# imironhead/ml_super_resolution

Measured on AMD Instinct MI355X. Metric: VDSR-20 training patches/sec (41x41, batch 256 per GPU); fwd HR megapixels/sec alongside, higher is better.
Workload: dtype f32; 1 GPU; BASELINE configs[2]: VDSR 20-layer 3x3x64 residual, RGB, batch 256x41x41 per GPU, fwd+bwd+TF-Adam, random-init weights; global_batch=256, patch=41, parallelism=dp1

## Files before the change

### ml_super_resolution_amd/csrc/conv_narrow.hip

```cpp
#include "launchers.h"
namespace srx {
typedef float f32x3 __attribute__((ext_vector_type(3)));
typedef unsigned u32x3v __attribute__((ext_vector_type(3)));

template <int CTRL>
__device__ __forceinline__ float dpp_add(float v) {
    const int moved = __builtin_amdgcn_update_dpp(0, __float_as_int(v), CTRL, 0xf, 0xf, false);
    return v + __int_as_float(moved);
}

struct PixWalk {
    int n, oh, ow;
    __device__ __forceinline__ void init(unsigned p, int OH, int OW) {
        const unsigned t = p / (unsigned)OW;
        ow = (int)(p - t * (unsigned)OW);
        n = (int)(t / (unsigned)OH);
        oh = (int)(t - (unsigned)n * (unsigned)OH);
    }
    __device__ __forceinline__ void step16(int OH, int OW) { step(16, OH, OW); }
    __device__ __forceinline__ void step(int d, int OH, int OW) {
        ow += d;
        while (ow >= OW) {
            ow -= OW;
            oh += 1;
            if (oh == OH) { oh = 0; n += 1; }
        }
    }
};
template <int KH, int KW>
__device__ __forceinline__ void tap_offsets(int (&off)[KH * KW], const PixWalk& q, bool live, int H, int W, int pad_t, int pad_l,
                                            int PB, int lane_b) {
    const int centre = ((q.n * H + q.oh - pad_t) * W + (q.ow - pad_l)) * PB + lane_b;
    bool rok[KH], cok[KW];
#pragma unroll
    for (int kh = 0; kh < KH; ++kh) rok[kh] = live && (unsigned)(q.oh + kh - pad_t) < (unsigned)H;
#pragma unroll
    for (int kw = 0; kw < KW; ++kw) cok[kw] = (unsigned)(q.ow + kw - pad_l) < (unsigned)W;
#pragma unroll
    for (int kh = 0; kh < KH; ++kh)
#pragma unroll
        for (int kw = 0; kw < KW; ++kw)
            off[kh * KW + kw] = (rok[kh] && cok[kw]) ? centre + (kh * W + kw) * PB : kOobOffset;
}

template <int KH, int KW, int CIN, int CO>
__global__ __launch_bounds__(256) void conv_narrow_kernel(const ConvArgs a, long total_px, int iters) {
    static_assert(CIN == 64, "16 lanes x 4 channels per pixel");
    constexpr int TAPS = KH * KW;
    const int c4 = threadIdx.x & 15;
    const int sub = threadIdx.x >> 4;
    float wr[TAPS][4][CO];
#pragma unroll
    for (int t = 0; t < TAPS; ++t)
#pragma unroll
        for (int e = 0; e < 4; ++e)
#pragma unroll
            for (int c = 0; c < CO; ++c) wr[t][e][c] = a.w[((size_t)t * CIN + 4 * c4 + e) * CO + c];
    float bias[CO];
#pragma unroll
    for (int c = 0; c < CO; ++c) bias[c] = a.bias ? a.bias[c] : 0.0f;
    const __amdgpu_buffer_rsrc_t xrs = __builtin_amdgcn_make_buffer_rsrc(const_cast<float*>(a.x), 0,
                                                                         a.N * a.H * a.W * CIN * 4, 0x00020000);
    const unsigned p0 = blockIdx.x * (unsigned)iters * 16u + sub;
    PixWalk q;
    q.init(p0 < (unsigned)total_px ? p0 : 0u, a.OH, a.OW);
    for (int it = 0; it < iters; ++it, q.step16(a.OH, a.OW)) {
        const unsigned p = p0 + (unsigned)it * 16u;
        const bool live = p < (unsigned)total_px;
        int off[TAPS];
        tap_offsets<KH, KW>(off, q, live, a.H, a.W, a.pad_t, a.pad_l, CIN * 4, 16 * c4);
        f32x4 v[TAPS];
#pragma unroll
        for (int tp = 0; tp < TAPS; ++tp)
            v[tp] = __builtin_bit_cast(f32x4, __builtin_amdgcn_raw_buffer_load_b128(xrs, off[tp], 0, 0));
        float acc[CO];
#pragma unroll
        for (int c = 0; c < CO; ++c) acc[c] = 0.0f;
#pragma unroll
        for (int tp = 0; tp < TAPS; ++tp)
#pragma unroll
            for (int e = 0; e < 4; ++e)
#pragma unroll
                for (int c = 0; c < CO; ++c) acc[c] = fmaf(v[tp][e], wr[tp][e][c], acc[c]);
#pragma unroll
        for (int c = 0; c < CO; ++c) {
            float r = acc[c];
            r = dpp_add<0xB1>(r);
            r = dpp_add<0x4E>(r);
            r = dpp_add<0x124>(r);
            r = dpp_add<0x128>(r);
            acc[c] = r;
        }
        if (live && c4 < CO) {
            float r = (c4 == 0) ? acc[0] : (c4 == 1 ? acc[1 < CO ? 1 : 0] : acc[2 < CO ? 2 : 0]);
            r = act_apply(r + ((c4 == 0) ? bias[0] : (c4 == 1 ? bias[1 < CO ? 1 : 0] : bias[2 < CO ? 2 : 0])), a.act);
            const size_t o = (size_t)p * CO + c4;
            if (a.skip) r += a.skip[o];
            if (a.post_relu) r = act_apply(r, a.post_relu);
            a.y[o] = r;
        }
    }
}

template <int KH, int KW, bool NOUT, int CW = 64>
__global__ __launch_bounds__(256) void wgrad_narrow_kernel(const WgradArgs a, long total_px, int iters) {
    constexpr int TAPS = KH * KW, CN = 3;
    constexpr int LPP = CW / 4;
    constexpr int PPI = 256 / LPP;
    constexpr int NB = NOUT ? CN : 4;
    constexpr int NV = TAPS * 4 * CN + NB;
    __shared__ float red[4 * NV * LPP];
    const int c4 = threadIdx.x & (LPP - 1);
    const int sub = threadIdx.x / LPP;
    const int wave = threadIdx.x >> 6;
    float acc[NV];
#pragma unroll
    for (int i = 0; i < NV; ++i) acc[i] = 0.0f;
    const __amdgpu_buffer_rsrc_t xrs = __builtin_amdgcn_make_buffer_rsrc(
        const_cast<float*>(a.x), 0, a.N * a.H * a.W * (NOUT ? CW : CN) * 4, 0x00020000);
    const __amdgpu_buffer_rsrc_t drs = __builtin_amdgcn_make_buffer_rsrc(
        const_cast<float*>(a.dpre), 0, a.N * a.OH * a.OW * (NOUT ? CN : CW) * 4, 0x00020000);
    const unsigned p0 = blockIdx.x * (unsigned)iters * (unsigned)PPI + sub;
    PixWalk q;
    q.init(p0 < (unsigned)total_px ? p0 : 0u, a.OH, a.OW);
    for (int it = 0; it < iters; ++it, q.step(PPI, a.OH, a.OW)) {
        const unsigned p = p0 + (unsigned)it * (unsigned)PPI;
        const bool live = p < (unsigned)total_px;
        int off[TAPS];
        tap_offsets<KH, KW>(off, q, live, a.H, a.W, a.pad_t, a.pad_l, (NOUT ? CW : CN) * 4, NOUT ? 16 * c4 : 0);
        if constexpr (NOUT) {
            const f32x3 d = __builtin_bit_cast(f32x3, __builtin_amdgcn_raw_buffer_load_b96(drs, live ? (int)(p * CN * 4) : kOobOffset, 0, 0));
            f32x4 v[TAPS];
#pragma unroll
            for (int tp = 0; tp < TAPS; ++tp)
                v[tp] = __builtin_bit_cast(f32x4, __builtin_amdgcn_raw_buffer_load_b128(xrs, off[tp], 0, 0));
#pragma unroll
            for (int tp = 0; tp < TAPS; ++tp)
#pragma unroll
                for (int e = 0; e < 4; ++e)
#pragma unroll
                    for (int c = 0; c < CN; ++c) acc[(tp * 4 + e) * CN + c] = fmaf(v[tp][e], d[c], acc[(tp * 4 + e) * CN + c]);
#pragma unroll
            for (int c = 0; c < CN; ++c) acc[TAPS * 4 * CN + c] += d[c];
        } else {
            const f32x4 d = __builtin_bit_cast(f32x4, __builtin_amdgcn_raw_buffer_load_b128(
                drs, live ? (int)((p * CW + 4 * c4) * 4) : kOobOffset, 0, 0));
            f32x3 v[TAPS];
#pragma unroll
            for (int tp = 0; tp < TAPS; ++tp)
                v[tp] = __builtin_bit_cast(f32x3, __builtin_amdgcn_raw_buffer_load_b96(xrs, off[tp], 0, 0));
#pragma unroll
            for (int tp = 0; tp < TAPS; ++tp)
#pragma unroll
                for (int cn = 0; cn < CN; ++cn)
#pragma unroll
                    for (int e = 0; e < 4; ++e) acc[(tp * CN + cn) * 4 + e] = fmaf(v[tp][cn], d[e], acc[(tp * CN + cn) * 4 + e]);
#pragma unroll
            for (int e = 0; e < 4; ++e) acc[TAPS * 4 * CN + e] += d[e];
        }
    }
#pragma unroll
    for (int i = 0; i < NV; ++i) {
        float r = acc[i];
#pragma unroll
        for (int o = LPP; o < 64; o <<= 1) r += __shfl_xor(r, o);
        if (sub % (64 / LPP) == 0) red[(wave * NV + i) * LPP + c4] = r;
    }
    __syncthreads();
    float* part = a.part + (size_t)blockIdx.x * a.part_stride;
    const int wn = TAPS * CW * CN;
    for (int q = threadIdx.x; q < NV * LPP; q += 256) {
        const int i = q / LPP, l = q % LPP;
        const float r = (red[(0 * NV + i) * LPP + l] + red[(1 * NV + i) * LPP + l]) +
                        (red[(2 * NV + i) * LPP + l] + red[(3 * NV + i) * LPP + l]);
        if (i < TAPS * 4 * CN) {
            int idx;
            if constexpr (NOUT) {
                const int c = i % CN, te = i / CN, e = te & 3, tp = te >> 2;
                idx = (tp * CW + 4 * l + e) * CN + c;
            } else {
                const int e = i & 3, tc = i >> 2;
                idx = tc * CW + 4 * l + e;
            }
            part[idx] = r;
        } else {
            const int b = i - TAPS * 4 * CN;
            if constexpr (NOUT) {
                if (l == 0) part[wn + b] = r;
            } else {
                part[wn + 4 * l + b] = r;
            }
        }
    }
}

bool launch_wgrad_narrow(const ConvKey& k, const WgradArgs& a, int grid, hipStream_t s, hipError_t* err) {
    if (k.kh != 3 || k.kw != 3) return false;
    const bool nout = a.Cin == 64 && a.Cout == 3, nin = a.Cin == 3 && a.Cout == 64, nin32 = a.Cin == 3 && a.Cout == 32;
    if (!nout && !nin && !nin32) return false;
    const long total = (long)a.N * a.OH * a.OW;
    if (total >= (1L << 31) - 4096 || (long)a.N * a.H * a.W * 64 * 4 >= (1L << 31) - 4096 || total * 64 * 4 >= (1L << 31) - 4096)
        return false;
    const long ppi = nin32 ? 32 : 16;
    const int iters = (int)((total + ppi * grid - 1) / (ppi * grid));
    if (nout)
        hipLaunchKernelGGL((wgrad_narrow_kernel<3, 3, true>), dim3(grid), dim3(256), 0, s, a, total, iters);
    else if (nin)
        hipLaunchKernelGGL((wgrad_narrow_kernel<3, 3, false>), dim3(grid), dim3(256), 0, s, a, total, iters);
    else
        hipLaunchKernelGGL((wgrad_narrow_kernel<3, 3, false, 32>), dim3(grid), dim3(256), 0, s, a, total, iters);
    *err = hipGetLastError();
    return true;
}

bool launch_conv_narrow(const ConvKey& k, const ConvArgs& a, hipStream_t s, hipError_t* err) {
    if (k.wt || a.Cout != 3 || a.mask) return false;
    if ((long)a.N * a.H * a.W * a.Cin * 4 >= (1L << 31) - 4096) return false;
    const long total = (long)a.N * a.OH * a.OW;
    int iters = 16;
    while (iters > 1 && total / (16L * iters) < 2048) iters >>= 1;
    const long blocks = (total + 16L * iters - 1) / (16L * iters);
    if (total >= (1L << 31) - 4096) return false;
    if (k.kh == 3 && k.kw == 3 && a.Cin == 64) {
        hipLaunchKernelGGL((conv_narrow_kernel<3, 3, 64, 3>), dim3((unsigned)blocks), dim3(256), 0, s, a, total, iters);
    } else {
        return false;
    }
    *err = hipGetLastError();
    return true;
}
}
```

Baseline: 19530 patches/s.

## Walk output rows in runs with sliding 3-column input window for narrow convs

Replaces the per-pixel narrow conv forward (64->3) and the 64<->3 wgrad kernels with row-run walkers. Each 16-lane group processes a contiguous run of up to 14 output pixels and keeps a rotating window of input columns, so each input column is loaded once per run instead of three times. Loads are software-prefetched two steps ahead. Inner FMAs use packed v_pk_fma_f32 written as inline asm, and outputs are written with buffer stores. This cuts redundant global loads and FMA instruction count, in exchange for more registers and hand-written asm with manual s_nop hazard handling.

```diff
diff --git a/ml_super_resolution_amd/csrc/conv_narrow.hip b/ml_super_resolution_amd/csrc/conv_narrow.hip
--- a/ml_super_resolution_amd/csrc/conv_narrow.hip
+++ b/ml_super_resolution_amd/csrc/conv_narrow.hip
@@ -1,4 +1,6 @@
 #include "launchers.h"
+#include <type_traits>
+#include <utility>
 namespace srx {
 typedef float f32x3 __attribute__((ext_vector_type(3)));
 typedef unsigned u32x3v __attribute__((ext_vector_type(3)));
@@ -43,62 +45,182 @@
             off[kh * KW + kw] = (rok[kh] && cok[kw]) ? centre + (kh * W + kw) * PB : kOobOffset;
 }
 
-template <int KH, int KW, int CIN, int CO>
-__global__ __launch_bounds__(256) void conv_narrow_kernel(const ConvArgs a, long total_px, int iters) {
-    static_assert(CIN == 64, "16 lanes x 4 channels per pixel");
-    constexpr int TAPS = KH * KW;
+constexpr int kRunMax = 14;
+
+struct RunPlan {
+    int nruns, steps;
+    unsigned total_runs;
+};
+inline RunPlan plan_runs(long rows, int OW) {
+    RunPlan r;
+    r.nruns = (OW + kRunMax - 1) / kRunMax;
+    r.steps = (OW + r.nruns - 1) / r.nruns;
+    r.total_runs = (unsigned)(rows * r.nruns);
+    return r;
+}
+
+struct Run {
+    int row, n, oh, ow0, len;
+    __device__ __forceinline__ void init(unsigned r, const RunPlan& rp, int OH, int OW) {
+        const bool live = r < rp.total_runs;
+        const unsigned rr = live ? r : 0u;
+        const unsigned rw = rr / (unsigned)rp.nruns;
+        row = (int)rw;
+        ow0 = (int)(rr - rw * (unsigned)rp.nruns) * rp.steps;
+        n = (int)(rw / (unsigned)OH);
+        oh = row - n * OH;
+        len = live ? min(rp.steps, OW - ow0) : 0;
+        if (len < 0) len = 0;
+    }
+};
+
+template <typename V>
+__device__ __forceinline__ V load_px(__amdgpu_buffer_rsrc_t rs, int off) {
+    if constexpr (sizeof(V) == 16)
+        return __builtin_bit_cast(V, __builtin_amdgcn_raw_buffer_load_b128(rs, off, 0, 0));
+    else
+        return __builtin_bit_cast(V, __builtin_amdgcn_raw_buffer_load_b96(rs, off, 0, 0));
+}
+
+template <typename V, int PB>
+struct ColWalk {
+    int o[3], iw;
+    bool rok[3];
+    __device__ __forceinline__ void init(const Run& q, int H, int W, int pad_t, int pad_l, int lane_b) {
+        iw = q.ow0 - pad_l;
+#pragma unroll
+        for (int kh = 0; kh < 3; ++kh) {
+            const int ih = q.oh + kh - pad_t;
+            rok[kh] = q.len > 0 && (unsigned)ih < (unsigned)H;
+            o[kh] = (int)((((unsigned)q.n * (unsigned)H + (unsigned)ih) * (unsigned)W + (unsigned)iw) * (unsigned)PB + (unsigned)lane_b);
+        }
+    }
+    __device__ __forceinline__ void next(__amdgpu_buffer_rsrc_t rs, int W, V (&col)[3], bool on = true) {
+        const bool cok = on && (unsigned)iw < (unsigned)W;
+#pragma unroll
+        for (int kh = 0; kh < 3; ++kh) {
+            col[kh] = load_px<V>(rs, (rok[kh] && cok) ? o[kh] : kOobOffset);
+            o[kh] += PB;
+        }
+        iw += 1;
+    }
+};
+
+template <int HALF, bool LAST = false>
+__device__ __forceinline__ void pk_fma_bcast(f32x2& acc, f32x2 a, f32x2 b) {
+    if constexpr (HALF == 0) {
+        if constexpr (LAST) asm volatile("v_pk_fma_f32 %0, %1, %2, %0 op_sel_hi:[0,1,1]\n\ts_nop 1" : "+v"(acc) : "v"(a), "v"(b));
+        else asm volatile("v_pk_fma_f32 %0, %1, %2, %0 op_sel_hi:[0,1,1]" : "+v"(acc) : "v"(a), "v"(b));
+    } else {
+        if constexpr (LAST) asm volatile("v_pk_fma_f32 %0, %1, %2, %0 op_sel:[1,0,0] op_sel_hi:[1,1,1]\n\ts_nop 1" : "+v"(acc) : "v"(a), "v"(b));
+        else asm volatile("v_pk_fma_f32 %0, %1, %2, %0 op_sel:[1,0,0] op_sel_hi:[1,1,1]" : "+v"(acc) : "v"(a), "v"(b));
+    }
+}
+__device__ __forceinline__ f32x2 lo2(f32x4 v) { return __builtin_shufflevector(v, v, 0, 1); }
+__device__ __forceinline__ f32x2 hi2(f32x4 v) { return __builtin_shufflevector(v, v, 2, 3); }
+__device__ __forceinline__ f32x2 lo2(f32x3 v) { return __builtin_shufflevector(v, v, 0, 1); }
+__device__ __forceinline__ f32x2 hi2(f32x3 v) { return __builtin_shufflevector(v, v, 2, -1); }
+
+__device__ __forceinline__ void loads_issued() { asm volatile("" ::: "memory"); }
+
+constexpr int kAhead = 2;
+constexpr int kSlots = 3 + kAhead;
+template <int S>
+using StepPhase = std::integral_constant<int, S>;
+template <typename F, int... I>
+__device__ __forceinline__ void walk_steps_impl(int steps, F&& f, std::integer_sequence<int, I...>) {
+    for (int s = 0;; s += kSlots) {
+        bool done = false;
+        ((done = done || (f(StepPhase<I>{}, s + I), s + I + 1 >= steps)), ...);
+        if (done) break;
+    }
+}
+template <typename F>
+__device__ __forceinline__ void walk_steps(int steps, F&& f) {
+    walk_steps_impl(steps, f, std::make_integer_sequence<int, kSlots>{});
+}
+
+__global__ __launch_bounds__(256) void conv_narrow_rows_kernel(const ConvArgs a, const RunPlan rp, int iters) {
+    constexpr int PB = 64 * 4;
     const int c4 = threadIdx.x & 15;
     const int sub = threadIdx.x >> 4;
-    float wr[TAPS][4][CO];
-#pragma unroll
-    for (int t = 0; t < TAPS; ++t)
-#pragma unroll
-        for (int e = 0; e < 4; ++e)
-#pragma unroll
-            for (int c = 0; c < CO; ++c) wr[t][e][c] = a.w[((size_t)t * CIN + 4 * c4 + e) * CO + c];
-    float bias[CO];
-#pragma unroll
-    for (int c = 0; c < CO; ++c) bias[c] = a.bias ? a.bias[c] : 0.0f;
-    const __amdgpu_buffer_rsrc_t xrs = __builtin_amdgcn_make_buffer_rsrc(const_cast<float*>(a.x), 0,
-                                                                         a.N * a.H * a.W * CIN * 4, 0x00020000);
-    const unsigned p0 = blockIdx.x * (unsigned)iters * 16u + sub;
-    PixWalk q;
-    q.init(p0 < (unsigned)total_px ? p0 : 0u, a.OH, a.OW);
-    for (int it = 0; it < iters; ++it, q.step16(a.OH, a.OW)) {
-        const unsigned p = p0 + (unsigned)it * 16u;
-        const bool live = p < (unsigned)total_px;
-        int off[TAPS];
-        tap_offsets<KH, KW>(off, q, live, a.H, a.W, a.pad_t, a.pad_l, CIN * 4, 16 * c4);
-        f32x4 v[TAPS];
-#pragma unroll
-        for (int tp = 0; tp < TAPS; ++tp)
-            v[tp] = __builtin_bit_cast(f32x4, __builtin_amdgcn_raw_buffer_load_b128(xrs, off[tp], 0, 0));
-        float acc[CO];
-#pragma unroll
-        for (int c = 0; c < CO; ++c) acc[c] = 0.0f;
-#pragma unroll
-        for (int tp = 0; tp < TAPS; ++tp)
-#pragma unroll
-            for (int e = 0; e < 4; ++e)
-#pragma unroll
-                for (int c = 0; c < CO; ++c) acc[c] = fmaf(v[tp][e], wr[tp][e][c], acc[c]);
-#pragma unroll
-        for (int c = 0; c < CO; ++c) {
-            float r = acc[c];
-            r = dpp_add<0xB1>(r);
-            r = dpp_add<0x4E>(r);
-            r = dpp_add<0x124>(r);
-            r = dpp_add<0x128>(r);
-            acc[c] = r;
-        }
-        if (live && c4 < CO) {
-            float r = (c4 == 0) ? acc[0] : (c4 == 1 ? acc[1 < CO ? 1 : 0] : acc[2 < CO ? 2 : 0]);
-            r = act_apply(r + ((c4 == 0) ? bias[0] : (c4 == 1 ? bias[1 < CO ? 1 : 0] : bias[2 < CO ? 2 : 0])), a.act);
-            const size_t o = (size_t)p * CO + c4;
-            if (a.skip) r += a.skip[o];
+    f32x2 w01[9][4];
+    float w2[9][4];
+#pragma unroll
+    for (int t = 0; t < 9; ++t)
+#pragma unroll
+        for (int e = 0; e < 4; ++e) {
+            const float* wp = a.w + ((size_t)t * 64 + 4 * c4 + e) * 3;
+            w01[t][e] = f32x2{wp[0], wp[1]};
+            w2[t][e] = wp[2];
+        }
+    const float bias_l = (a.bias && c4 < 3) ? a.bias[c4] : 0.0f;
+    const int ybytes = a.N * a.OH * a.OW * 3 * 4;
+    const __amdgpu_buffer_rsrc_t xrs = __builtin_amdgcn_make_buffer_rsrc(const_cast<float*>(a.x), 0, a.N * a.H * a.W * PB, 0x00020000);
+    const __amdgpu_buffer_rsrc_t yrs = __builtin_amdgcn_make_buffer_rsrc(a.y, 0, ybytes, 0x00020000);
+    const __amdgpu_buffer_rsrc_t srs = __builtin_amdgcn_make_buffer_rsrc(const_cast<float*>(a.skip), 0, a.skip ? ybytes : 0, 0x00020000);
+    for (int it = 0; it < iters; ++it) {
+        Run q;
+        q.init((blockIdx.x * (unsigned)iters + (unsigned)it) * 16u + sub, rp, a.OH, a.OW);
+        ColWalk<f32x4, PB> cw;
+        cw.init(q, a.H, a.W, a.pad_t, a.pad_l, 16 * c4);
+        f32x4 win[kSlots][3];
+#pragma unroll
+        for (int c = 0; c < kSlots - 1; ++c) cw.next(xrs, a.W, win[c], c < rp.steps + 2);
+        int yo = ((q.row * a.OW + q.ow0) * 3 + c4) * 4;
+        int left = (c4 < 3) ? q.len : 0;
+        int so_ahead = yo, left_ahead = left;
+        auto next_skip = [&]() {
+            const float v = __builtin_bit_cast(float, __builtin_amdgcn_raw_buffer_load_b32(srs, left_ahead > 0 ? so_ahead : kOobOffset, 0, 0));
+            so_ahead += 12;
+            left_ahead -= 1;
+            return v;
+        };
+        float sk[kSlots];
+#pragma unroll
+        for (int c = 0; c < kAhead; ++c) sk[c] = next_skip();
+        walk_steps(rp.steps, [&](auto phase, int s) {
+            constexpr int S = decltype(phase)::value;
+            const int so = left > 0 ? yo : kOobOffset;
+            sk[(S + kAhead) % kSlots] = next_skip();
+            cw.next(xrs, a.W, win[(S + kSlots - 1) % kSlots], s + kAhead < rp.steps);
+            loads_issued();
+            f32x2 acc01 = {0.0f, 0.0f};
+            float acc2 = 0.0f;
+#pragma unroll
+            for (int kh = 0; kh < 3; ++kh)
+#pragma unroll
+                for (int kw = 0; kw < 3; ++kw) {
+                    const f32x4 v = win[(S + kw) % kSlots][kh];
+                    const int tp = kh * 3 + kw;
+                    pk_fma_bcast<0>(acc01, lo2(v), w01[tp][0]);
+                    acc2 = fmaf(v[0], w2[tp][0], acc2);
+                    pk_fma_bcast<1>(acc01, lo2(v), w01[tp][1]);
+                    acc2 = fmaf(v[1], w2[tp][1], acc2);
+                    pk_fma_bcast<0>(acc01, hi2(v), w01[tp][2]);
+                    acc2 = fmaf(v[2], w2[tp][2], acc2);
+                    if (tp == 8) pk_fma_bcast<1, true>(acc01, hi2(v), w01[tp][3]);
+                    else pk_fma_bcast<1>(acc01, hi2(v), w01[tp][3]);
+                    acc2 = fmaf(v[3], w2[tp][3], acc2);
+                }
+            float r3[3] = {acc01[0], acc01[1], acc2};
+#pragma unroll
+            for (int c = 0; c < 3; ++c) {
+                float r = r3[c];
+                r = dpp_add<0xB1>(r);
+                r = dpp_add<0x4E>(r);
+                r = dpp_add<0x124>(r);
+                r = dpp_add<0x128>(r);
+                r3[c] = r;
+            }
+            float r = (c4 == 0) ? r3[0] : (c4 == 1 ? r3[1] : r3[2]);
+            r = act_apply(r + bias_l, a.act);
+            r = a.skip ? r + sk[S] : r;
             if (a.post_relu) r = act_apply(r, a.post_relu);
-            a.y[o] = r;
-        }
+            __builtin_amdgcn_raw_buffer_store_b32(__builtin_bit_cast(unsigned, r), yrs, so, 0, 0);
+            yo += 12;
+            left -= 1;
+        });
     }
 }
 
@@ -194,6 +316,104 @@
     }
 }
 
+template <bool NOUT>
+__global__ __launch_bounds__(256) void wgrad_narrow_rows_kernel(const WgradArgs a, const RunPlan rp, int iters) {
+    constexpr int TAPS = 9, CN = 3, CW = 64, LPP = 16;
+    constexpr int NB = NOUT ? CN : 4;
+    constexpr int NV = TAPS * 4 * CN + NB;
+    constexpr int PBX = (NOUT ? CW : CN) * 4, PBD = (NOUT ? CN : CW) * 4;
+    using VX = typename std::conditional<NOUT, f32x4, f32x3>::type;
+    using VD = typename std::conditional<NOUT, f32x3, f32x4>::type;
+    __shared__ float red[4 * NV * LPP];
+    const int c4 = threadIdx.x & (LPP - 1);
+    const int sub = threadIdx.x / LPP;
+    const int wave = threadIdx.x >> 6;
+    f32x2 acc[TAPS * CN * 2];
+    float accb[4] = {0.0f, 0.0f, 0.0f, 0.0f};
+#pragma unroll
+    for (int i = 0; i < TAPS * CN * 2; ++i) acc[i] = f32x2{0.0f, 0.0f};
+    const __amdgpu_buffer_rsrc_t xrs = __builtin_amdgcn_make_buffer_rsrc(const_cast<float*>(a.x), 0, a.N * a.H * a.W * PBX, 0x00020000);
+    const __amdgpu_buffer_rsrc_t drs = __builtin_amdgcn_make_buffer_rsrc(const_cast<float*>(a.dpre), 0, a.N * a.OH * a.OW * PBD, 0x00020000);
+    for (int it = 0; it < iters; ++it) {
+        Run q;
+        q.init((blockIdx.x * (unsigned)iters + (unsigned)it) * 16u + sub, rp, a.OH, a.OW);
+        ColWalk<VX, PBX> cw;
+        cw.init(q, a.H, a.W, a.pad_t, a.pad_l, NOUT ? 16 * c4 : 0);
+        int dof = (q.row * a.OW + q.ow0) * PBD + (NOUT ? 0 : 16 * c4);
+        int left = q.len;
+        auto next_d = [&]() {
+            const VD d = load_px<VD>(drs, left > 0 ? dof : kOobOffset);
+            dof += PBD;
+            left -= 1;
+            return d;
+        };
+        VX win[kSlots][3];
+        VD dd[kSlots];
+#pragma unroll
+        for (int c = 0; c < kSlots - 1; ++c) cw.next(xrs, a.W, win[c], c < rp.steps + 2);
+#pragma unroll
+        for (int c = 0; c < kAhead; ++c) dd[c] = next_d();
+        walk_steps(rp.steps, [&](auto phase, int s) {
+            constexpr int S = decltype(phase)::value;
+            cw.next(xrs, a.W, win[(S + kSlots - 1) % kSlots], s + kAhead < rp.steps);
+            dd[(S + kAhead) % kSlots] = next_d();
+            loads_issued();
+            const VD d = dd[S];
+#pragma unroll
+            for (int kh = 0; kh < 3; ++kh)
+#pragma unroll
+                for (int kw = 0; kw < 3; ++kw) {
+                    const VX v = win[(S + kw) % kSlots][kh];
+                    const int t3 = (kh * 3 + kw) * CN;
+#pragma unroll
+                    for (int c = 0; c < CN; ++c) {
+                        f32x2& a0 = acc[(t3 + c) * 2], &a1 = acc[(t3 + c) * 2 + 1];
+                        if constexpr (NOUT) {
+                            if (c == 0) { pk_fma_bcast<0>(a0, lo2(d), lo2(v)); pk_fma_bcast<0>(a1, lo2(d), hi2(v)); }
+                            else if (c == 1) { pk_fma_bcast<1>(a0, lo2(d), lo2(v)); pk_fma_bcast<1>(a1, lo2(d), hi2(v)); }
+                            else { pk_fma_bcast<0>(a0, hi2(d), lo2(v)); pk_fma_bcast<0>(a1, hi2(d), hi2(v)); }
+                        } else {
+                            if (c == 0) { pk_fma_bcast<0>(a0, lo2(v), lo2(d)); pk_fma_bcast<0>(a1, lo2(v), hi2(d)); }
+                            else if (c == 1) { pk_fma_bcast<1>(a0, lo2(v), lo2(d)); pk_fma_bcast<1>(a1, lo2(v), hi2(d)); }
+                            else { pk_fma_bcast<0>(a0, hi2(v), lo2(d)); pk_fma_bcast<0>(a1, hi2(v), hi2(d)); }
+                        }
+                    }
+                }
+#pragma unroll
+            for (int b = 0; b < NB; ++b) accb[b] += d[b];
+        });
+    }
+#pragma unroll
+    for (int i = 0; i < NV; ++i) {
+        float r = (i < TAPS * 4 * CN) ? acc[i >> 1][i & 1] : accb[(i - TAPS * 4 * CN) & 3];
+        r += __shfl_xor(r, 16);
+        r += __shfl_xor(r, 32);
+        if ((sub & 3) == 0) red[(wave * NV + i) * LPP + c4] = r;
+    }
+    __syncthreads();
+    float* part = a.part + (size_t)blockIdx.x * a.part_stride;
+    const int wn = TAPS * CW * CN;
+    for (int q = threadIdx.x; q < NV * LPP; q += 256) {
+        const int i = q / LPP, l = q % LPP;
+        const float r = (red[(0 * NV + i) * LPP + l] + red[(1 * NV + i) * LPP + l]) +
+                        (red[(2 * NV + i) * LPP + l] + red[(3 * NV + i) * LPP + l]);
+        if (i < TAPS * 4 * CN) {
+            const int e = i & 3, tc = i >> 2;
+            if constexpr (NOUT)
+                part[((tc / CN) * CW + 4 * l + e) * CN + tc % CN] = r;
+            else
+                part[tc * CW + 4 * l + e] = r;
+        } else {
+            const int b = i - TAPS * 4 * CN;
+            if constexpr (NOUT) {
+                if (l == 0) part[wn + b] = r;
+            } else {
+                part[wn + 4 * l + b] = r;
+            }
+        }
+    }
+}
+
 bool launch_wgrad_narrow(const ConvKey& k, const WgradArgs& a, int grid, hipStream_t s, hipError_t* err) {
     if (k.kh != 3 || k.kw != 3) return false;
     const bool nout = a.Cin == 64 && a.Cout == 3, nin = a.Cin == 3 && a.Cout == 64, nin32 = a.Cin == 3 && a.Cout == 32;
@@ -201,14 +421,18 @@
     const long total = (long)a.N * a.OH * a.OW;
     if (total >= (1L << 31) - 4096 || (long)a.N * a.H * a.W * 64 * 4 >= (1L << 31) - 4096 || total * 64 * 4 >= (1L << 31) - 4096)
         return false;
-    const long ppi = nin32 ? 32 : 16;
-    const int iters = (int)((total + ppi * grid - 1) / (ppi * grid));
-    if (nout)
-        hipLaunchKernelGGL((wgrad_narrow_kernel<3, 3, true>), dim3(grid), dim3(256), 0, s, a, total, iters);
-    else if (nin)
-        hipLaunchKernelGGL((wgrad_narrow_kernel<3, 3, false>), dim3(grid), dim3(256), 0, s, a, total, iters);
-    else
+    if (nin32) {
+        const long ppi = 32;
+        const int iters = (int)((total + ppi * grid - 1) / (ppi * grid));
         hipLaunchKernelGGL((wgrad_narrow_kernel<3, 3, false, 32>), dim3(grid), dim3(256), 0, s, a, total, iters);
+    } else {
+        const RunPlan rp = plan_runs((long)a.N * a.OH, a.OW);
+        const int iters = (int)(((long)rp.total_runs + 16L * grid - 1) / (16L * grid));
+        if (nout)
+            hipLaunchKernelGGL((wgrad_narrow_rows_kernel<true>), dim3(grid), dim3(256), 0, s, a, rp, iters);
+        else
+            hipLaunchKernelGGL((wgrad_narrow_rows_kernel<false>), dim3(grid), dim3(256), 0, s, a, rp, iters);
+    }
     *err = hipGetLastError();
     return true;
 }
@@ -217,15 +441,13 @@
     if (k.wt || a.Cout != 3 || a.mask) return false;
     if ((long)a.N * a.H * a.W * a.Cin * 4 >= (1L << 31) - 4096) return false;
     const long total = (long)a.N * a.OH * a.OW;
-    int iters = 16;
-    while (iters > 1 && total / (16L * iters) < 2048) iters >>= 1;
-    const long blocks = (total + 16L * iters - 1) / (16L * iters);
     if (total >= (1L << 31) - 4096) return false;
-    if (k.kh == 3 && k.kw == 3 && a.Cin == 64) {
-        hipLaunchKernelGGL((conv_narrow_kernel<3, 3, 64, 3>), dim3((unsigned)blocks), dim3(256), 0, s, a, total, iters);
-    } else {
-        return false;
-    }
+    if (k.kh != 3 || k.kw != 3 || a.Cin != 64) return false;
+    const RunPlan rp = plan_runs((long)a.N * a.OH, a.OW);
+    int iters = 4;
+    while (iters > 1 && (long)rp.total_runs / (16L * iters) < 768) iters >>= 1;
+    const long blocks = ((long)rp.total_runs + 16L * iters - 1) / (16L * iters);
+    hipLaunchKernelGGL(conv_narrow_rows_kernel, dim3((unsigned)blocks), dim3(256), 0, s, a, rp, iters);
     *err = hipGetLastError();
     return true;
 }
```

Result: no change. 19510 patches/s (-0.1%).
